# donydchen/matchnerf

Hardware: AMD Instinct MI355X
Metric: rendered rays/sec (3-view, 64 samples/ray) (higher is better)
Workload: dtype f32; 1 GPU

## Files before the change

matchnerf_amd/csrc/api.cpp:

```cpp
#include <string.h>
#include <stdarg.h>
#include <stdio.h>
#include <stdlib.h>

#include <mutex>

#include "common.hpp"
#include "launch_plan.hpp"

static thread_local char g_err[512] = "";

void mnerf_set_error(const char* fmt, ...) {
  va_list ap;
  va_start(ap, fmt);
  vsnprintf(g_err, sizeof(g_err), fmt, ap);
  va_end(ap);
}

extern "C" int mnerf_abi_version(void) { return MNERF_ABI_VERSION; }
extern "C" const char* mnerf_last_error(void) { return g_err; }

extern "C" int64_t mnerf_struct_size(int32_t which) {
  switch (which) {
    case 0: return (int64_t)sizeof(mnerf_view);
// ... 43 lines not shown
  c.height = c.tgt_height = rays->height, c.width = c.tgt_width = rays->width;
  c.near_ = rays->near_, c.far_ = rays->far_;
  c.strat_u = rays->strat_u;
  *out = c;
  return MNERF_OK;
}

static int env_int(const char* name, int dflt) {
  const char* e = getenv(name);
  return (e && *e) ? atoi(e) : dflt;
}

static mnerf_tuning read_tuning() {
  mnerf_tuning t;
  t.decoder_grid = env_int("MNERF_DECODER_GRID", 512);
  t.decoder_stagger = env_int("MNERF_DECODER_STAGGER", 16);
  t.decoder_stagger_mode = env_int("MNERF_DECODER_STAGGER_MODE", 0);
  t.cv_variant = env_int("MNERF_CV_VARIANT", 3);
  t.cv_mm = env_int("MNERF_CV_MM", 1);
  t.cv_mm_spw = env_int("MNERF_CV_MM_SPW", 4);
  t.cv_uvpair = env_int("MNERF_CV_UVPAIR", -1);
  t.cv_pair_block = env_int("MNERF_CV_PAIR_BLOCK", -1);
  t.cv_grid = env_int("MNERF_CV_GRID", 0);
  t.wa_min4 = env_int("MNERF_WA_MIN4", 200);
  t.wa_xcd = env_int("MNERF_WA_XCD", 1);
  t.render_fused = env_int("MNERF_RENDER_FUSED", 0);
  t.decoder_pp = env_int("MNERF_DECODER_PP", 1);
  t.decoder_pp_grid = env_int("MNERF_DECODER_PP_GRID", 256);
  t.decoder_pp_max_s = env_int("MNERF_DECODER_PP_MAX_S", 256);
  return t;
}

static mnerf_tuning g_tuning = read_tuning();
static std::mutex g_tuning_lock;
mnerf_tuning mnerf_tune() {
  std::lock_guard<std::mutex> hold(g_tuning_lock);
  return g_tuning;
}

extern "C" int mnerf_debug_set_knob(const char* name, int value, int* old_value) {
  std::lock_guard<std::mutex> hold(g_tuning_lock);
  struct Knob { const char* name; int* slot; };
  const Knob knobs[] = {{"decoder_pp", &g_tuning.decoder_pp}, {"decoder_pp_grid", &g_tuning.decoder_pp_grid},
                        {"decoder_pp_max_s", &g_tuning.decoder_pp_max_s}, {"decoder_grid", &g_tuning.decoder_grid},
                        {"cv_variant", &g_tuning.cv_variant}, {"cv_mm", &g_tuning.cv_mm}, {"cv_mm_spw", &g_tuning.cv_mm_spw}, {"cv_uvpair", &g_tuning.cv_uvpair}, {"cv_pair_block", &g_tuning.cv_pair_block}, {"cv_grid", &g_tuning.cv_grid},
                        {"render_fused", &g_tuning.render_fused}, {"wa_min4", &g_tuning.wa_min4}};
  for (const Knob& k : knobs)
    if (name && strcmp(name, k.name) == 0) {
      if (old_value) *old_value = *k.slot;
      *k.slot = value;
      return MNERF_OK;
    }
  mnerf_set_error("mnerf_debug_set_knob: unknown knob '%s'", name ? name : "(null)");
  return MNERF_E_RANGE;
}

extern "C" int mnerf_debug_launch_plan(const char* what, const int64_t* args, int32_t n_args, int32_t* plan, int32_t n_plan) {
  MNERF_REQUIRE(what && args && plan, MNERF_E_NULL, "mnerf_debug_launch_plan: NULL argument");
  struct Planner { const char* name; int (*fn)(const int64_t*, int32_t, int32_t*, int32_t); };
  const Planner planners[] = {{"conv2d", mnerf_plan_conv2d}, {"conv_gemm", mnerf_plan_conv_gemm}, {"conv_wgrad", mnerf_plan_conv_wgrad},
                              {"instance_norm", mnerf_plan_instance_norm}, {"instance_norm_backward", mnerf_plan_instance_norm},
                              {"window_attention", mnerf_plan_window_attention}};
  for (const Planner& p : planners)
    if (strcmp(what, p.name) == 0) return p.fn(args, n_args, plan, n_plan);
  mnerf_set_error("mnerf_debug_launch_plan: unknown dispatcher '%s'", what);
  return MNERF_E_RANGE;
}

bool mnerf_once_per_device(std::atomic<unsigned long long>& mask) {
  int dev = 0;
  (void)hipGetDevice(&dev);
  const unsigned long long bit = 1ull << (dev & 63);
  return (mask.fetch_or(bit, std::memory_order_relaxed) & bit) == 0;
}
```

matchnerf_amd/csrc/qkv.hip:

```cpp
#include "wa_common.hpp"

#define QKV_NW 2
#define QKV_SEG_FLOATS (32 * 256)
#define QKV_C 128

struct QkvParams {
  const float* xq;
  const float* xkv;
  float* out[3];
  const float* wstream;
  int n_tokens, seq_len, n_seq, kv_swap;
  int ew[3];
};

__device__ __forceinline__ int qkv_load_split(const float* __restrict__ row, PartsH (&xp)[8]) {
  float x[64];
  float amax = 0.0f;
#pragma unroll
  for (int t = 0; t < 8; ++t) {
    const float4 a = *reinterpret_cast<const float4*>(row + 16 * t), b = *reinterpret_cast<const float4*>(row + 16 * t + 4);
    x[8 * t + 0] = a.x; x[8 * t + 1] = a.y; x[8 * t + 2] = a.z; x[8 * t + 3] = a.w;
    x[8 * t + 4] = b.x; x[8 * t + 5] = b.y; x[8 * t + 6] = b.z; x[8 * t + 7] = b.w;
  }
#pragma unroll
// ... 76 lines not shown
  const float* xkv;
  float* q;
  u32x4* img;
  int* rec;
  const float* wstream;
  WinGeom G;
  int n_batch, n_tiles, total_tiles, kv_swap;
  int ew[3];
};

template <int NS>
__device__ __forceinline__ void ksteps_presplit_swapped(f32x16 (&acc)[4], unsigned base_lds, int lane, const PartsH* x) {
  lds_u32x4_cptr a = (lds_u32x4_cptr)(size_t)base_lds + lane;
  u32x4 ch = a[0], cl = a[64];
#pragma unroll
  for (int u = 0; u < NS; ++u) {
#pragma unroll
    for (int m = 0; m < 4; ++m) {
      const int i = u * 4 + m;
      const int nx = (i + 1 < NS * 4) ? (i + 1) * 128 : i * 128;
      const u32x4 nh = a[nx], nl = a[nx + 64];
      __builtin_amdgcn_sched_barrier(0);
      const f16x8 wh = __builtin_bit_cast(f16x8, ch), wl = __builtin_bit_cast(f16x8, cl);
      acc[m] = mfma16h(x[u].lo, wh, acc[m]);
      acc[m] = mfma16h(x[u].hi, wl, acc[m]);
      acc[m] = mfma16h(x[u].hi, wh, acc[m]);
      __builtin_amdgcn_sched_barrier(0);
      ch = nh;
      cl = nl;
    }
  }
}

__global__ __launch_bounds__(QKV_NW * 64, 2) void qkv_images_kernel(QkvImgParams P) {
  extern __shared__ __attribute__((aligned(16))) float qkv_smem[];
  const unsigned buf0 = (unsigned)(size_t)(__attribute__((address_space(3))) float*)qkv_smem;
  const int tid = threadIdx.x, lane = tid & 63;
  const int wave = __builtin_amdgcn_readfirstlane(tid >> 6);
  const int n = lane & 31, hl = lane >> 5;
  auto stage = [&](int seg) {
    const float* src = P.wstream + (size_t)seg * QKV_SEG_FLOATS + lane * 4;
    const unsigned dst = buf0 + (unsigned)(seg & 1) * (QKV_SEG_FLOATS * 4u);
    glds_segment(src, dst, QKV_SEG_FLOATS / 256, wave, QKV_NW);
  };
  stage(0);

  const WinGeom& G = P.G;
  const int t_raw = blockIdx.x * QKV_NW + wave;
  const bool tile_ok = t_raw < P.total_tiles;
  const int tile = tile_ok ? t_raw : P.total_tiles - 1;
  const int gwin = tile / P.n_tiles, kt = tile - gwin * P.n_tiles;
  const int n_win = G.splits * G.splits;
  const int b = gwin / n_win, win = gwin - b * n_win;
  const int wy = win / G.splits, wx = win - wy * G.splits;
  const int li = kt * WA_KT + n;
  const bool key_ok = li < G.Lw;
  int region_unused;
  const int tok = win_token(G, wy, wx, key_ok ? li : G.Lw - 1, region_unused);
  int b_kv = b;
  if (P.kv_swap) {
    b_kv = b + (P.n_batch >> 1);
    if (b_kv >= P.n_batch) b_kv -= P.n_batch;
  }
  const size_t hw = (size_t)G.h * G.w;
  const bool same_rows = !P.kv_swap && P.xkv == P.xq;

  PartsH xp[8];
  int eg = qkv_load_split(P.xq + ((size_t)b * hw + tok) * QKV_C + 8 * hl, xp);
  segment_wait();
  __syncthreads();

  u32x4* img = P.img + (size_t)tile * (WA_IMG_BYTES / 16) + lane;
  int ek = 0, ev = 0;
  int seg = 0;
#pragma unroll 1
  for (int proj = 0; proj < 3; ++proj) {
    if (proj == 1 && !same_rows) eg = qkv_load_split(P.xkv + ((size_t)b_kv * hw + tok) * QKV_C + 8 * hl, xp);
    f32x16 acc[4];
#pragma unroll
    for (int m = 0; m < 4; ++m) acc[m] = (f32x16)(0.0f);
#pragma unroll
    for (int half = 0; half < 2; ++half, ++seg) {
      if (seg + 1 < 6) stage(seg + 1);
      const unsigned cur = buf0 + (unsigned)(seg & 1) * (QKV_SEG_FLOATS * 4u);
      if (proj == 2) ksteps_presplit_swapped<4>(acc, cur, lane, xp + 4 * half);
      else ksteps_presplit<4, 4>(acc, cur, lane, xp + 4 * half);
      segment_wait();
      __syncthreads();
    }
    if (proj == 0) {
      if (tile_ok && key_ok) {
        const float cm = pow2i(-(P.ew[0] + eg));
        float* dst = P.q + ((size_t)b * hw + tok) * QKV_C + 4 * hl;
#pragma unroll
        for (int m = 0; m < 4; ++m)
#pragma unroll
          for (int g = 0; g < 4; ++g)
            *reinterpret_cast<float4*>(dst + 32 * m + 8 * g) =
                make_float4(acc[m][4 * g] * cm, acc[m][4 * g + 1] * cm, acc[m][4 * g + 2] * cm, acc[m][4 * g + 3] * cm);
      }
      continue;
    }
    if (proj == 1) {
      const float cm = pow2i(-(P.ew[1] + eg));
#pragma unroll
      for (int m = 0; m < 4; ++m)
#pragma unroll
        for (int r = 0; r < 16; ++r) acc[m][r] *= cm;
    } else {
#pragma unroll
      for (int r = 0; r < 16; ++r) {
        const int key = (r & 3) + 8 * (r >> 2) + 4 * hl;
        const int eg_key = __shfl(eg, key, 64);
        const float cm = pow2i(-(P.ew[2] + eg_key));
#pragma unroll
        for (int m = 0; m < 4; ++m) acc[m][r] *= cm;
      }
    }
    float tmax = 0.0f;
#pragma unroll
    for (int m = 0; m < 4; ++m)
#pragma unroll
      for (int r = 0; r < 16; ++r) tmax = fmaxf(tmax, fabsf(acc[m][r]));
#pragma unroll
    for (int off = 32; off > 0; off >>= 1) tmax = fmaxf(tmax, __shfl_xor(tmax, off, 64));
    const int et = gain_exp(tmax);
    const float mt = pow2i(et);
    if (proj == 1) {
      ek = et;
      if (tile_ok) {
#pragma unroll
        for (int t = 0; t < 8; ++t) {
          float v8[8];
#pragma unroll
          for (int j = 0; j < 8; ++j) v8[j] = acc[t >> 1][8 * (t & 1) + j];
          const PartsH kp = split8h(v8, mt);
          img[(2 * t) * 64] = __builtin_bit_cast(u32x4, kp.hi);
          img[(2 * t + 1) * 64] = __builtin_bit_cast(u32x4, kp.lo);
        }
      }
    } else {
      ev = et;
      if (tile_ok) {
#pragma unroll
        for (int t = 0; t < 2; ++t)
#pragma unroll
          for (int m = 0; m < 4; ++m) {
            float v8[8];
#pragma unroll
            for (int j = 0; j < 8; ++j) v8[j] = acc[m][8 * t + j];
            const PartsH vp = split8h(v8, mt);
            img[(WA_IMG_VOFF / 64 + 2 * (4 * t + m)) * 64] = __builtin_bit_cast(u32x4, vp.hi);
            img[(WA_IMG_VOFF / 64 + 2 * (4 * t + m) + 1) * 64] = __builtin_bit_cast(u32x4, vp.lo);
          }
      }
    }
  }
  if (tile_ok) {
    int* rec = P.rec + WA_REC_INTS * (size_t)tile;
    wa_store_regions(G, wy, wx, kt, lane, rec);
    if (lane == 0) {
      rec[0] = ek;
      rec[1] = ev;
    }
  }
}

extern "C" int mnerf_qkv_window_images(const float* wstream, const int32_t* ew, const float* x_q, const float* x_kv,
                                       int32_t kv_swap, float* q, void* workspace, size_t workspace_bytes, int32_t batch,
                                       int32_t h, int32_t w, int32_t num_splits, int32_t shifted, void* stream) {
  const char* who = "mnerf_qkv_window_images";
  WinGeom G;
  int do_shift;
  if (const int rc = wa_geometry(who, batch, h, w, num_splits, shifted, G, do_shift)) return rc;
  MNERF_REQUIRE(!kv_swap || batch % 2 == 0, MNERF_E_RANGE, "%s: kv_swap needs an even number of sequences, got %d", who, batch);
  if (batch == 0) return MNERF_OK;
  MNERF_REQUIRE(wstream && ew && x_q && x_kv && q, MNERF_E_NULL, "%s: NULL buffer", who);
  MNERF_REQUIRE(mnerf_aligned16(wstream) && mnerf_aligned16(x_q) && mnerf_aligned16(x_kv) && mnerf_aligned16(q), MNERF_E_ALIGN,
                "%s: buffers must be 16-byte aligned", who);
  const size_t need = wa_workspace_bytes(batch, h, w, num_splits);
  MNERF_REQUIRE(workspace && mnerf_aligned16(workspace), MNERF_E_ALIGN, "%s: workspace NULL or not 16-byte aligned", who);
  MNERF_REQUIRE(workspace_bytes >= need, MNERF_E_RANGE, "%s: workspace %zu bytes < %zu", who, workspace_bytes, need);
  QkvImgParams p;
  p.xq = x_q;
  p.xkv = x_kv;
  p.q = q;
  p.wstream = wstream;
  p.G = G;
  p.n_batch = batch;
  p.n_tiles = (G.Lw + WA_KT - 1) / WA_KT;
  p.total_tiles = batch * num_splits * num_splits * p.n_tiles;
  p.kv_swap = kv_swap ? 1 : 0;
  p.img = reinterpret_cast<u32x4*>(workspace);
  p.rec = reinterpret_cast<int*>(reinterpret_cast<char*>(workspace) + (size_t)p.total_tiles * WA_IMG_BYTES);
  for (int i = 0; i < 3; ++i) p.ew[i] = ew[i];
  const size_t lds = 2 * QKV_SEG_FLOATS * sizeof(float);
  static std::atomic<unsigned long long> attr{0};
  if (mnerf_once_per_device(attr))
    (void)hipFuncSetAttribute((const void*)qkv_images_kernel, hipFuncAttributeMaxDynamicSharedMemorySize, (int)lds);
  hipLaunchKernelGGL(qkv_images_kernel, dim3((p.total_tiles + QKV_NW - 1) / QKV_NW), dim3(QKV_NW * 64), lds, (hipStream_t)stream, p);
  return mnerf_check_launch(who);
}

extern "C" int64_t mnerf_qkv_wstream_floats(void) { return 6 * (int64_t)QKV_SEG_FLOATS; }

extern "C" int mnerf_qkv_projection(const float* wstream, const int32_t* ew, const float* x_q, const float* x_kv,
                                    int32_t kv_swap, float* q, float* k, float* v, int32_t n_seq, int32_t seq_len,
                                    void* stream) {
  const char* who = "mnerf_qkv_projection";
  MNERF_REQUIRE(n_seq >= 0 && seq_len >= 1 && (long long)n_seq * seq_len <= 0x7fffffffLL, MNERF_E_RANGE,
                "%s: n_seq=%d seq_len=%d", who, n_seq, seq_len);
  MNERF_REQUIRE(!kv_swap || n_seq % 2 == 0, MNERF_E_RANGE, "%s: kv_swap needs an even number of sequences, got %d", who, n_seq);
  if (n_seq == 0) return MNERF_OK;
  MNERF_REQUIRE(wstream && ew && x_q && x_kv && q && k && v, MNERF_E_NULL, "%s: NULL buffer", who);
  MNERF_REQUIRE(mnerf_aligned16(wstream) && mnerf_aligned16(x_q) && mnerf_aligned16(x_kv) && mnerf_aligned16(q) &&
                    mnerf_aligned16(k) && mnerf_aligned16(v),
                MNERF_E_ALIGN, "%s: buffers must be 16-byte aligned", who);
  QkvParams p;
  p.xq = x_q;
  p.xkv = x_kv;
  p.out[0] = q;
  p.out[1] = k;
  p.out[2] = v;
  p.wstream = wstream;
  p.n_tokens = n_seq * seq_len;
  p.seq_len = seq_len;
  p.n_seq = n_seq;
  p.kv_swap = kv_swap ? 1 : 0;
  for (int i = 0; i < 3; ++i) p.ew[i] = ew[i];
  const size_t lds = 2 * QKV_SEG_FLOATS * sizeof(float);
  static std::atomic<unsigned long long> attr{0};
  if (mnerf_once_per_device(attr))
    (void)hipFuncSetAttribute((const void*)qkv_kernel, hipFuncAttributeMaxDynamicSharedMemorySize, (int)lds);
// ... 5 lines not shown
```

matchnerf_amd/csrc/wa_common.hpp:

```cpp
#pragma once
#include "split_f16.hpp"

#define WA_C 128
#define WA_KT 32
#define WA_IMG_BYTES 32768
#define WA_IMG_VOFF 1024
#define WA_REC_INTS 8

struct WinGeom {
  int h, w, wh, ww, sh, sw, splits, Lw;
};

__device__ __forceinline__ int win_token(const WinGeom& G, int wy, int wx, int li, int& region) {
  const int ly = li / G.ww, lx = li - ly * G.ww;
  const int ry = wy * G.wh + ly, rx = wx * G.ww + lx;
  int oy = ry + G.sh, ox = rx + G.sw;
  if (oy >= G.h) oy -= G.h;
  if (ox >= G.w) ox -= G.w;
  const int regy = (ry >= G.h - G.wh) + (ry >= G.h - G.sh);
  const int regx = (rx >= G.w - G.ww) + (rx >= G.w - G.sw);
  region = regy * 3 + regx;
  return oy * G.w + ox;
}

__device__ __forceinline__ void wa_store_regions(const WinGeom& G, int wy, int wx, int kt, int lane, int* rec) {
  const int n = lane & 31;
  int li = kt * WA_KT + n, region;
  if (li >= G.Lw) li = G.Lw - 1;
  (void)win_token(G, wy, wx, li, region);
  unsigned nib = (unsigned)region << (4 * (n & 7));
  nib |= __shfl_xor(nib, 1, 64);
  nib |= __shfl_xor(nib, 2, 64);
  nib |= __shfl_xor(nib, 4, 64);
  if (lane < 32 && (lane & 7) == 0) rec[2 + (lane >> 3)] = (int)nib;
}

static inline int wa_geometry(const char* who, int32_t batch, int32_t h, int32_t w, int32_t num_splits, int32_t shifted,
                       WinGeom& G, int& do_shift) {
  MNERF_REQUIRE(batch >= 0 && h >= 1 && w >= 1 && num_splits >= 1, MNERF_E_RANGE, "%s: batch=%d h=%d w=%d splits=%d",
                who, batch, h, w, num_splits);
  MNERF_REQUIRE(h % num_splits == 0 && w % num_splits == 0, MNERF_E_RANGE, "%s: %dx%d not divisible into %d splits",
                who, h, w, num_splits);
  MNERF_REQUIRE(batch <= 65535 && num_splits * num_splits <= 65535, MNERF_E_RANGE, "%s: grid too large", who);
  G.h = h;
// ... 19 lines not shown
```

matchnerf_amd/csrc/window_attention.hip:

```cpp
#include <stdlib.h>

#include "wa_common.hpp"
#include "launch_plan.hpp"

__device__ __forceinline__ void wa_glds16(const float* gsrc, unsigned lds_byte_addr) {
  unsigned keep;
  asm volatile(
      "s_mov_b32 %0, m0\n\t"
      "s_mov_b32 m0, %2\n\t"
      "s_nop 0\n\t"
      "global_load_lds_dwordx4 %1, off\n\t"
      "s_mov_b32 m0, %0"
      : "=&s"(keep)
      : "v"(gsrc), "s"(lds_byte_addr)
      : "memory");
}

__device__ __forceinline__ void wa_glds16x4(const float* gsrc, unsigned lds_byte_addr) {
  unsigned keep;
  asm volatile(
      "s_mov_b32 %0, m0\n\t"
      "s_mov_b32 m0, %2\n\t"
      "s_nop 0\n\t"
      "global_load_lds_dwordx4 %1, off\n\t"
// ... 465 lines not shown
      for (int r = 0; r < 16; ++r) o[m][r] *= corr;
#pragma unroll
    for (int t = 0; t < 2; ++t) {
      float pv[8];
#pragma unroll
      for (int j = 0; j < 8; ++j) pv[j] = s[8 * t + j];
      const PartsH pp = split8h(pv, 16384.0f);
#pragma unroll
      for (int m = 0; m < 4; ++m) {
        const PartsH vp = split8h(vv[t][m], mv);
        o[m] = mfma16h(vp.hi, pp.lo, o[m]);
        o[m] = mfma16h(vp.lo, pp.hi, o[m]);
        o[m] = mfma16h(vp.hi, pp.hi, o[m]);
      }
    }
    asm volatile("s_waitcnt vmcnt(0)" ::: "memory");
    __syncthreads();
  }
  if (q_ok) {
    const float inv_l = pow2i(-(ev_run + 14)) / l_run;
    float* dst = out + seq_base + (size_t)q_tok * WA_C;
#pragma unroll
    for (int m = 0; m < 4; ++m)
#pragma unroll
      for (int g4 = 0; g4 < 4; ++g4) {
        const float4 t = make_float4(o[m][4 * g4] * inv_l, o[m][4 * g4 + 1] * inv_l,
                                     o[m][4 * g4 + 2] * inv_l, o[m][4 * g4 + 3] * inv_l);
        *reinterpret_cast<float4*>(dst + m * 32 + 8 * g4 + 4 * hl) = t;
      }
  }
}


__global__ __launch_bounds__(64) void wa_presplit_kernel(const float* __restrict__ k, const float* __restrict__ v,
                                                         u32x4* __restrict__ img, int* __restrict__ gains, WinGeom G) {
  const int lane = threadIdx.x, n = lane & 31, hl = lane >> 5;
  const int kt = blockIdx.x, win = blockIdx.y, b = blockIdx.z;
  const int wy = win / G.splits, wx = win - wy * G.splits;
  const size_t seq_base = (size_t)b * G.h * G.w * WA_C;
  const size_t tile = ((size_t)b * gridDim.y + win) * gridDim.x + kt;
  u32x4* dst = img + tile * (WA_IMG_BYTES / 16) + lane;
  int reg_unused;
  int ek, ev;
  {
    int li = kt * WA_KT + n;
    if (li >= G.Lw) li = G.Lw - 1;
    const int tok = win_token(G, wy, wx, li, reg_unused);
    const float4* src = reinterpret_cast<const float4*>(k + seq_base + (size_t)tok * WA_C + hl * 8);
    float kv[64];
    float kmax = 0.0f;
#pragma unroll
    for (int t = 0; t < 8; ++t) {
      const float4 a = src[4 * t], c = src[4 * t + 1];
      kv[8 * t + 0] = a.x; kv[8 * t + 1] = a.y; kv[8 * t + 2] = a.z; kv[8 * t + 3] = a.w;
      kv[8 * t + 4] = c.x; kv[8 * t + 5] = c.y; kv[8 * t + 6] = c.z; kv[8 * t + 7] = c.w;
    }
#pragma unroll
    for (int i = 0; i < 64; ++i) kmax = fmaxf(kmax, fabsf(kv[i]));
#pragma unroll
    for (int off = 32; off > 0; off >>= 1) kmax = fmaxf(kmax, __shfl_xor(kmax, off, 64));
    ek = gain_exp(kmax);
    const float mk = pow2i(ek);
#pragma unroll
    for (int t = 0; t < 8; ++t) {
      float v8[8];
#pragma unroll
      for (int j = 0; j < 8; ++j) v8[j] = kv[8 * t + j];
      const PartsH kp = split8h(v8, mk);
      dst[(2 * t) * 64] = __builtin_bit_cast(u32x4, kp.hi);
      dst[(2 * t + 1) * 64] = __builtin_bit_cast(u32x4, kp.lo);
    }
  }
  {
    float vv[2][4][8];
    float vmax = 0.0f;
#pragma unroll
    for (int t = 0; t < 2; ++t)
#pragma unroll
      for (int j = 0; j < 8; ++j) {
        const int r = 8 * t + j;
        int li = kt * WA_KT + (r & 3) + 8 * (r >> 2) + 4 * hl;
        if (li >= G.Lw) li = G.Lw - 1;
        const int tok = win_token(G, wy, wx, li, reg_unused);
        const float* row = v + seq_base + (size_t)tok * WA_C + n;
#pragma unroll
        for (int m = 0; m < 4; ++m) {
          const float x = row[32 * m];
          vv[t][m][j] = x;
          vmax = fmaxf(vmax, fabsf(x));
        }
      }
#pragma unroll
    for (int off = 32; off > 0; off >>= 1) vmax = fmaxf(vmax, __shfl_xor(vmax, off, 64));
    ev = gain_exp(vmax);
    const float mv = pow2i(ev);
#pragma unroll
    for (int t = 0; t < 2; ++t)
#pragma unroll
      for (int m = 0; m < 4; ++m) {
        const PartsH vp = split8h(vv[t][m], mv);
        dst[(WA_IMG_VOFF / 64 + 2 * (4 * t + m)) * 64] = __builtin_bit_cast(u32x4, vp.hi);
        dst[(WA_IMG_VOFF / 64 + 2 * (4 * t + m) + 1) * 64] = __builtin_bit_cast(u32x4, vp.lo);
      }
  }
  int* rec = gains + WA_REC_INTS * tile;
  wa_store_regions(G, wy, wx, kt, lane, rec);
  if (lane == 0) {
    rec[0] = ek;
    rec[1] = ev;
  }
}

__device__ __forceinline__ void wa_halves(float x, float& lo, float& hi) {
  unsigned a = __builtin_bit_cast(unsigned, x), b = a;
  asm("s_nop 1\n\tv_permlane32_swap_b32_e32 %0, %1" : "+v"(a), "+v"(b));
  lo = __builtin_bit_cast(float, a);
  hi = __builtin_bit_cast(float, b);
}

template <int NQW>
__device__ __forceinline__ void wa_stage_image(const u32x4* __restrict__ img_tile, unsigned lds_base, int wave, int lane) {
  for (int piece = wave; piece < WA_IMG_BYTES / 1024; piece += NQW)
    wa_glds16(reinterpret_cast<const float*>(img_tile + piece * 64 + lane),
              __builtin_amdgcn_readfirstlane(lds_base + (unsigned)piece * 1024u));
}

template <int NQW, bool STATS = false>
__global__ __launch_bounds__(NQW * 64, 2) void window_attention_pre_kernel(
    const float* __restrict__ q, const u32x4* __restrict__ img, const int* __restrict__ gains,
    float* __restrict__ out, WinGeom G, int shifted, float scale, int n_batch, int xcd_map, unsigned long long* tl) {
  extern __shared__ __attribute__((aligned(16))) float wa_smem[];
  const unsigned smem0 = (unsigned)(size_t)(__attribute__((address_space(3))) float*)wa_smem;
  const int tid = threadIdx.x, lane = tid & 63;
  const int wave = __builtin_amdgcn_readfirstlane(tid >> 6);
  const int n = lane & 31, hl = lane >> 5;
  const int n_win = G.splits * G.splits;
// ... 217 lines not shown
    WA_STAMP(5);
    ra = ra_next;
    rb = rb_next;
  }
#undef WA_SLOT
#ifdef MNERF_TIMELINE
  if (tl && lane == 0 && blockIdx.x < 64)
    for (int i = 0; i < 6; ++i) tl[(blockIdx.x * NQW + wave) * 6 + i] = tph[i];
#endif
  if (q_ok) {
    const float inv_l = pow2i(-(ev_run + 14)) / l_run;
    float* dst = out + seq_base + (size_t)q_tok * WA_C;
#pragma unroll
    for (int m = 0; m < 4; ++m)
#pragma unroll
      for (int g4 = 0; g4 < 4; ++g4) {
        const float4 t = make_float4(o[m][4 * g4] * inv_l, o[m][4 * g4 + 1] * inv_l,
                                     o[m][4 * g4 + 2] * inv_l, o[m][4 * g4 + 3] * inv_l);
        *reinterpret_cast<float4*>(dst + m * 32 + 8 * g4 + 4 * hl) = t;
      }
#ifndef MNERF_TIMELINE
    if constexpr (STATS) {
      if (hl == 0) {
        float* st = reinterpret_cast<float*>(tl);
        const size_t tok = (size_t)b * G.h * G.w + q_tok, n_tok = (size_t)n_batch * G.h * G.w;
        st[tok] = m_run;
        st[n_tok + tok] = l_run;
      }
    }
#endif
  }
}

extern "C" size_t mnerf_window_attention_workspace_bytes(int32_t batch, int32_t h, int32_t w, int32_t num_splits) {
  return wa_workspace_bytes(batch, h, w, num_splits);
}

static bool wa_take_four(int Lw, int n_win, int batch) {
  const long long wgs4 = (long long)((Lw + 127) / 128) * n_win * batch;
  return wgs4 >= mnerf_tune().wa_min4;
}

int mnerf_plan_window_attention(const int64_t* a, int32_t n_args, int32_t* plan, int32_t n_plan) {
  const char* who = "mnerf_debug_launch_plan(window_attention)";
  MNERF_REQUIRE(n_args == 4 && n_plan >= 1, MNERF_E_RANGE, "%s: takes 4 arguments and fills 1 value, got %d and %d", who, n_args, n_plan);
  MNERF_REQUIRE(a[0] >= 1 && a[0] <= 65535 && a[1] >= 1 && a[2] >= 1 && a[1] <= 0x7fff && a[2] <= 0x7fff && a[3] >= 1 && a[3] <= 255,
                MNERF_E_RANGE, "%s: batch=%lld h=%lld w=%lld splits=%lld", who, (long long)a[0], (long long)a[1], (long long)a[2], (long long)a[3]);
  MNERF_REQUIRE(a[1] % a[3] == 0 && a[2] % a[3] == 0, MNERF_E_RANGE, "%s: %lldx%lld not divisible into %lld splits", who, (long long)a[1],
                (long long)a[2], (long long)a[3]);
  plan[0] = wa_take_four((int)((a[1] / a[3]) * (a[2] / a[3])), (int)(a[3] * a[3]), (int)a[0]) ? 4 : 2;
  return MNERF_OK;
}

static int wa_launch_main(const char* who, const float* q, float* out, const WinGeom& G, int do_shift, int32_t batch,
                          int32_t num_splits, void* workspace, hipStream_t st, float* row_stats = nullptr) {
  const int n_tiles = (G.Lw + WA_KT - 1) / WA_KT;
  const int n_win = num_splits * num_splits;
  const u32x4* img = reinterpret_cast<const u32x4*>(workspace);
  const int* gains = reinterpret_cast<const int*>(reinterpret_cast<const char*>(workspace) + (size_t)batch * n_win * n_tiles * WA_IMG_BYTES);
  const float scale = 1.0f / sqrtf((float)WA_C);
  const size_t lds = 2 * WA_IMG_BYTES;
  static std::atomic<unsigned long long> attr{0};
  if (mnerf_once_per_device(attr)) {
    (void)hipFuncSetAttribute((const void*)window_attention_pre_kernel<4>, hipFuncAttributeMaxDynamicSharedMemorySize, (int)lds);
    (void)hipFuncSetAttribute((const void*)window_attention_pre_kernel<2>, hipFuncAttributeMaxDynamicSharedMemorySize, (int)lds);
    (void)hipFuncSetAttribute((const void*)window_attention_pre_kernel<4, true>, hipFuncAttributeMaxDynamicSharedMemorySize, (int)lds);
    (void)hipFuncSetAttribute((const void*)window_attention_pre_kernel<2, true>, hipFuncAttributeMaxDynamicSharedMemorySize, (int)lds);
  }
  unsigned long long* tl = nullptr;
#ifdef MNERF_TIMELINE
  if (const char* e = getenv("MNERF_WA_TIMELINE_PTR")) tl = (unsigned long long*)strtoull(e, nullptr, 0);
#endif
  const long long win_groups = ((long long)n_win * batch + 7) / 8;
  const int xcd = mnerf_tune().wa_xcd;
  const bool four = wa_take_four(G.Lw, n_win, batch);
  const int n_qb = four ? (G.Lw + 127) / 128 : (G.Lw + 63) / 64;
  const dim3 grid((unsigned)(8 * win_groups * n_qb));
#ifndef MNERF_TIMELINE
  if (row_stats) {
    unsigned long long* sp = reinterpret_cast<unsigned long long*>(row_stats);
    if (four)
      hipLaunchKernelGGL((window_attention_pre_kernel<4, true>), grid, dim3(256), lds, st, q, img, gains, out, G, do_shift, scale, batch, xcd, sp);
    else
      hipLaunchKernelGGL((window_attention_pre_kernel<2, true>), grid, dim3(128), lds, st, q, img, gains, out, G, do_shift, scale, batch, xcd, sp);
    return mnerf_check_launch(who);
  }
#else
  MNERF_REQUIRE(!row_stats, MNERF_E_UNSUPPORTED, "%s: no row statistics in the timeline build", who);
#endif
  if (four)
    hipLaunchKernelGGL(window_attention_pre_kernel<4>, grid, dim3(256), lds, st, q, img, gains, out, G, do_shift, scale, batch, xcd, tl);
  else
    hipLaunchKernelGGL(window_attention_pre_kernel<2>, grid, dim3(128), lds, st, q, img, gains, out, G, do_shift, scale, batch, xcd, tl);
  return mnerf_check_launch(who);
}

static int wa_check_workspace(const char* who, const void* workspace, size_t workspace_bytes, int32_t batch, int32_t h,
                              int32_t w, int32_t num_splits) {
  const size_t need = wa_workspace_bytes(batch, h, w, num_splits);
  MNERF_REQUIRE(workspace && mnerf_aligned16(workspace), MNERF_E_ALIGN, "%s: workspace NULL or not 16-byte aligned", who);
  MNERF_REQUIRE(workspace_bytes >= need, MNERF_E_RANGE, "%s: workspace %zu bytes < %zu", who, workspace_bytes, need);
  return MNERF_OK;
}

static int wa_presplit_impl(const char* who, const float* q, const float* k, const float* v, float* out, float* row_stats,
                            int32_t batch, int32_t h, int32_t w, int32_t num_splits, int32_t shifted, void* workspace,
                            size_t workspace_bytes, void* stream) {
  MNERF_REQUIRE(q && k && v && out, MNERF_E_NULL, "%s: NULL buffer", who);
  MNERF_REQUIRE(mnerf_aligned16(q) && mnerf_aligned16(k) && mnerf_aligned16(v) && mnerf_aligned16(out), MNERF_E_ALIGN,
                "%s: buffers must be 16-byte aligned", who);
  WinGeom G;
  int do_shift;
  if (const int rc = wa_geometry(who, batch, h, w, num_splits, shifted, G, do_shift)) return rc;
  if (batch == 0) return MNERF_OK;
  if (const int rc = wa_check_workspace(who, workspace, workspace_bytes, batch, h, w, num_splits)) return rc;
  const int n_tiles = (G.Lw + WA_KT - 1) / WA_KT;
  const int n_win = num_splits * num_splits;
  u32x4* img = reinterpret_cast<u32x4*>(workspace);
  int* gains = reinterpret_cast<int*>(reinterpret_cast<char*>(workspace) + (size_t)batch * n_win * n_tiles * WA_IMG_BYTES);
  hipStream_t st = (hipStream_t)stream;
  hipLaunchKernelGGL(wa_presplit_kernel, dim3(n_tiles, n_win, batch), dim3(64), 0, st, k, v, img, gains, G);
  return wa_launch_main(who, q, out, G, do_shift, batch, num_splits, workspace, st, row_stats);
}

extern "C" int mnerf_window_attention_presplit(const float* q, const float* k, const float* v, float* out,
                                               int32_t batch, int32_t h, int32_t w, int32_t num_splits, int32_t shifted,
                                               void* workspace, size_t workspace_bytes, void* stream) {
  return wa_presplit_impl("mnerf_window_attention_presplit", q, k, v, out, nullptr, batch, h, w, num_splits, shifted, workspace,
                          workspace_bytes, stream);
}

extern "C" int mnerf_window_attention_presplit_stats(const float* q, const float* k, const float* v, float* out, float* row_stats,
                                                     int32_t batch, int32_t h, int32_t w, int32_t num_splits, int32_t shifted,
                                                     void* workspace, size_t workspace_bytes, void* stream) {
  const char* who = "mnerf_window_attention_presplit_stats";
  MNERF_REQUIRE(row_stats, MNERF_E_NULL, "%s: row_stats is NULL", who);
  return wa_presplit_impl(who, q, k, v, out, row_stats, batch, h, w, num_splits, shifted, workspace, workspace_bytes, stream);
}

extern "C" int mnerf_window_attention_images(const float* q, float* out, int32_t batch, int32_t h, int32_t w,
                                             int32_t num_splits, int32_t shifted, const void* workspace,
                                             size_t workspace_bytes, void* stream) {
  const char* who = "mnerf_window_attention_images";
  MNERF_REQUIRE(q && out, MNERF_E_NULL, "%s: NULL buffer", who);
  MNERF_REQUIRE(mnerf_aligned16(q) && mnerf_aligned16(out), MNERF_E_ALIGN, "%s: buffers must be 16-byte aligned", who);
  WinGeom G;
  int do_shift;
  if (const int rc = wa_geometry(who, batch, h, w, num_splits, shifted, G, do_shift)) return rc;
  if (batch == 0) return MNERF_OK;
  if (const int rc = wa_check_workspace(who, workspace, workspace_bytes, batch, h, w, num_splits)) return rc;
  return wa_launch_main(who, q, out, G, do_shift, batch, num_splits, const_cast<void*>(workspace), (hipStream_t)stream);
}

extern "C" int mnerf_window_attention(const float* q, const float* k, const float* v, float* out,
                                      int32_t batch, int32_t h, int32_t w, int32_t num_splits,
                                      int32_t shifted, int32_t math, void* stream) {
  MNERF_REQUIRE(q && k && v && out, MNERF_E_NULL, "mnerf_window_attention: NULL buffer");
  MNERF_REQUIRE(mnerf_aligned16(q) && mnerf_aligned16(k) && mnerf_aligned16(v) && mnerf_aligned16(out),
                MNERF_E_ALIGN, "mnerf_window_attention: buffers must be 16-byte aligned");
  MNERF_REQUIRE(batch >= 0 && h >= 1 && w >= 1 && num_splits >= 1, MNERF_E_RANGE,
                "mnerf_window_attention: batch=%d h=%d w=%d splits=%d", batch, h, w, num_splits);
  MNERF_REQUIRE(h % num_splits == 0 && w % num_splits == 0, MNERF_E_RANGE,
                "mnerf_window_attention: %dx%d not divisible into %d splits", h, w, num_splits);
  MNERF_REQUIRE(batch <= 65535 && num_splits * num_splits <= 65535, MNERF_E_RANGE,
                "mnerf_window_attention: grid too large");
  MNERF_REQUIRE(math == MNERF_WA_SPLIT_BF16 || math == MNERF_WA_EXACT_F32 || math == MNERF_WA_SPLIT_F16, MNERF_E_UNSUPPORTED,
                "mnerf_window_attention: math=%d", math);
  if (batch == 0) return MNERF_OK;
  WinGeom G;
  G.h = h;
  G.w = w;
  G.splits = num_splits;
  G.wh = h / num_splits;
  G.ww = w / num_splits;
  const int do_shift = (shifted && num_splits > 1) ? 1 : 0;
  G.sh = do_shift ? G.wh / 2 : 0;
  G.sw = do_shift ? G.ww / 2 : 0;
  G.Lw = G.wh * G.ww;
  const float scale = 1.0f / sqrtf((float)WA_C);
  hipStream_t st = (hipStream_t)stream;
  const size_t lds = 4 * WA_KT * WA_C * sizeof(float);
  const bool split = math == MNERF_WA_SPLIT_BF16;
  const bool split_h = math == MNERF_WA_SPLIT_F16;
  static std::atomic<unsigned long long> attr_f32{0}, attr_split{0}, attr_split_h{0};
// ... 32 lines not shown
```

Before: 13.21 million rays/s.

## Add 16-row MFMA window-attention kernel with matching K/V image layout

Adds a window-attention kernel that uses 16x16x32 f16 MFMA with 16-row query fragments instead of the prior 32-row form. The K/V image written by the presplit and QKV projection kernels gets a matching 16-row layout. The path is on by default (MNERF_WA_ROWS=16) whenever the 128-query workgroup path is chosen. The aim is better MFMA shape efficiency and finer-grained softmax reductions, at the cost of new layout code that every producer must keep consistent.

```diff
diff --git a/matchnerf_amd/csrc/api.cpp b/matchnerf_amd/csrc/api.cpp
--- a/matchnerf_amd/csrc/api.cpp
+++ b/matchnerf_amd/csrc/api.cpp
@@ -99,7 +99,12 @@
 }
 
 static mnerf_tuning g_tuning = read_tuning();
+static int g_wa_rows = env_int("MNERF_WA_ROWS", 16);
 static std::mutex g_tuning_lock;
+int mnerf_wa_rows() {
+  std::lock_guard<std::mutex> hold(g_tuning_lock);
+  return g_wa_rows;
+}
 mnerf_tuning mnerf_tune() {
   std::lock_guard<std::mutex> hold(g_tuning_lock);
   return g_tuning;
@@ -111,7 +116,7 @@
   const Knob knobs[] = {{"decoder_pp", &g_tuning.decoder_pp}, {"decoder_pp_grid", &g_tuning.decoder_pp_grid},
                         {"decoder_pp_max_s", &g_tuning.decoder_pp_max_s}, {"decoder_grid", &g_tuning.decoder_grid},
                         {"cv_variant", &g_tuning.cv_variant}, {"cv_mm", &g_tuning.cv_mm}, {"cv_mm_spw", &g_tuning.cv_mm_spw}, {"cv_uvpair", &g_tuning.cv_uvpair}, {"cv_pair_block", &g_tuning.cv_pair_block}, {"cv_grid", &g_tuning.cv_grid},
-                        {"render_fused", &g_tuning.render_fused}, {"wa_min4", &g_tuning.wa_min4}};
+                        {"render_fused", &g_tuning.render_fused}, {"wa_min4", &g_tuning.wa_min4}, {"wa_rows", &g_wa_rows}};
   for (const Knob& k : knobs)
     if (name && strcmp(name, k.name) == 0) {
       if (old_value) *old_value = *k.slot;
diff --git a/matchnerf_amd/csrc/qkv.hip b/matchnerf_amd/csrc/qkv.hip
--- a/matchnerf_amd/csrc/qkv.hip
+++ b/matchnerf_amd/csrc/qkv.hip
@@ -132,6 +132,7 @@
   }
 }
 
+template <int LAYOUT>
 __global__ __launch_bounds__(QKV_NW * 64, 2) void qkv_images_kernel(QkvImgParams P) {
   extern __shared__ __attribute__((aligned(16))) float qkv_smem[];
   const unsigned buf0 = (unsigned)(size_t)(__attribute__((address_space(3))) float*)qkv_smem;
@@ -170,7 +171,8 @@
   segment_wait();
   __syncthreads();
 
-  u32x4* img = P.img + (size_t)tile * (WA_IMG_BYTES / 16) + lane;
+  u32x4* img_tile = P.img + (size_t)tile * (WA_IMG_BYTES / 16);
+  u32x4* img = img_tile + lane;
   int ek = 0, ev = 0;
   int seg = 0;
 #pragma unroll 1
@@ -235,8 +237,14 @@
 #pragma unroll
           for (int j = 0; j < 8; ++j) v8[j] = acc[t >> 1][8 * (t & 1) + j];
           const PartsH kp = split8h(v8, mt);
-          img[(2 * t) * 64] = __builtin_bit_cast(u32x4, kp.hi);
-          img[(2 * t + 1) * 64] = __builtin_bit_cast(u32x4, kp.lo);
+          if constexpr (LAYOUT == WA_IMG_ROWS16) {
+            u32x4* dst = img_tile + (2 * (4 * (n >> 4) + (t >> 1))) * 64 + (n & 15) + 16 * (2 * (t & 1) + hl);
+            dst[0] = __builtin_bit_cast(u32x4, kp.hi);
+            dst[64] = __builtin_bit_cast(u32x4, kp.lo);
+          } else {
+            img[(2 * t) * 64] = __builtin_bit_cast(u32x4, kp.hi);
+            img[(2 * t + 1) * 64] = __builtin_bit_cast(u32x4, kp.lo);
+          }
         }
       }
     } else {
@@ -247,11 +255,20 @@
 #pragma unroll
           for (int m = 0; m < 4; ++m) {
             float v8[8];
-#pragma unroll
-            for (int j = 0; j < 8; ++j) v8[j] = acc[m][8 * t + j];
-            const PartsH vp = split8h(v8, mt);
-            img[(WA_IMG_VOFF / 64 + 2 * (4 * t + m)) * 64] = __builtin_bit_cast(u32x4, vp.hi);
-            img[(WA_IMG_VOFF / 64 + 2 * (4 * t + m) + 1) * 64] = __builtin_bit_cast(u32x4, vp.lo);
+            if constexpr (LAYOUT == WA_IMG_ROWS16) {
+#pragma unroll
+              for (int j = 0; j < 8; ++j) v8[j] = acc[m][8 * (j >> 2) + 4 * t + (j & 3)];
+              const PartsH vp = split8h(v8, mt);
+              u32x4* dst = img_tile + (WA_IMG_VOFF / 64 + 2 * (2 * m + (n >> 4))) * 64 + (n & 15) + 16 * (2 * t + hl);
+              dst[0] = __builtin_bit_cast(u32x4, vp.hi);
+              dst[64] = __builtin_bit_cast(u32x4, vp.lo);
+            } else {
+#pragma unroll
+              for (int j = 0; j < 8; ++j) v8[j] = acc[m][8 * t + j];
+              const PartsH vp = split8h(v8, mt);
+              img[(WA_IMG_VOFF / 64 + 2 * (4 * t + m)) * 64] = __builtin_bit_cast(u32x4, vp.hi);
+              img[(WA_IMG_VOFF / 64 + 2 * (4 * t + m) + 1) * 64] = __builtin_bit_cast(u32x4, vp.lo);
+            }
           }
       }
     }
@@ -296,9 +313,15 @@
   for (int i = 0; i < 3; ++i) p.ew[i] = ew[i];
   const size_t lds = 2 * QKV_SEG_FLOATS * sizeof(float);
   static std::atomic<unsigned long long> attr{0};
-  if (mnerf_once_per_device(attr))
-    (void)hipFuncSetAttribute((const void*)qkv_images_kernel, hipFuncAttributeMaxDynamicSharedMemorySize, (int)lds);
-  hipLaunchKernelGGL(qkv_images_kernel, dim3((p.total_tiles + QKV_NW - 1) / QKV_NW), dim3(QKV_NW * 64), lds, (hipStream_t)stream, p);
+  if (mnerf_once_per_device(attr)) {
+    (void)hipFuncSetAttribute((const void*)qkv_images_kernel<WA_IMG_ROWS32>, hipFuncAttributeMaxDynamicSharedMemorySize, (int)lds);
+    (void)hipFuncSetAttribute((const void*)qkv_images_kernel<WA_IMG_ROWS16>, hipFuncAttributeMaxDynamicSharedMemorySize, (int)lds);
+  }
+  const dim3 grid((p.total_tiles + QKV_NW - 1) / QKV_NW);
+  if (wa_rows16(G.Lw, num_splits * num_splits, batch))
+    hipLaunchKernelGGL(qkv_images_kernel<WA_IMG_ROWS16>, grid, dim3(QKV_NW * 64), lds, (hipStream_t)stream, p);
+  else
+    hipLaunchKernelGGL(qkv_images_kernel<WA_IMG_ROWS32>, grid, dim3(QKV_NW * 64), lds, (hipStream_t)stream, p);
   return mnerf_check_launch(who);
 }
 
diff --git a/matchnerf_amd/csrc/wa_common.hpp b/matchnerf_amd/csrc/wa_common.hpp
--- a/matchnerf_amd/csrc/wa_common.hpp
+++ b/matchnerf_amd/csrc/wa_common.hpp
@@ -7,9 +7,19 @@
 #define WA_IMG_VOFF 1024
 #define WA_REC_INTS 8
 
+enum { WA_IMG_ROWS32 = 0, WA_IMG_ROWS16 = 1 };
+
 struct WinGeom {
   int h, w, wh, ww, sh, sw, splits, Lw;
 };
+
+static inline bool wa_take_four(int Lw, int n_win, int batch) {
+  const long long wgs4 = (long long)((Lw + 127) / 128) * n_win * batch;
+  return wgs4 >= mnerf_tune().wa_min4;
+}
+
+int mnerf_wa_rows();
+static inline bool wa_rows16(int Lw, int n_win, int batch) { return mnerf_wa_rows() != 32 && wa_take_four(Lw, n_win, batch); }
 
 __device__ __forceinline__ int win_token(const WinGeom& G, int wy, int wx, int li, int& region) {
   const int ly = li / G.ww, lx = li - ly * G.ww;
diff --git a/matchnerf_amd/csrc/window_attention.hip b/matchnerf_amd/csrc/window_attention.hip
--- a/matchnerf_amd/csrc/window_attention.hip
+++ b/matchnerf_amd/csrc/window_attention.hip
@@ -521,9 +521,11 @@
 }
 
 
+template <int LAYOUT>
 __global__ __launch_bounds__(64) void wa_presplit_kernel(const float* __restrict__ k, const float* __restrict__ v,
                                                          u32x4* __restrict__ img, int* __restrict__ gains, WinGeom G) {
   const int lane = threadIdx.x, n = lane & 31, hl = lane >> 5;
+  const int c16 = lane & 15, g16 = lane >> 4;
   const int kt = blockIdx.x, win = blockIdx.y, b = blockIdx.z;
   const int wy = win / G.splits, wx = win - wy * G.splits;
   const size_t seq_base = (size_t)b * G.h * G.w * WA_C;
@@ -532,17 +534,34 @@
   int reg_unused;
   int ek, ev;
   {
-    int li = kt * WA_KT + n;
-    if (li >= G.Lw) li = G.Lw - 1;
-    const int tok = win_token(G, wy, wx, li, reg_unused);
-    const float4* src = reinterpret_cast<const float4*>(k + seq_base + (size_t)tok * WA_C + hl * 8);
     float kv[64];
     float kmax = 0.0f;
-#pragma unroll
-    for (int t = 0; t < 8; ++t) {
-      const float4 a = src[4 * t], c = src[4 * t + 1];
-      kv[8 * t + 0] = a.x; kv[8 * t + 1] = a.y; kv[8 * t + 2] = a.z; kv[8 * t + 3] = a.w;
-      kv[8 * t + 4] = c.x; kv[8 * t + 5] = c.y; kv[8 * t + 6] = c.z; kv[8 * t + 7] = c.w;
+    if constexpr (LAYOUT == WA_IMG_ROWS16) {
+#pragma unroll
+      for (int kb = 0; kb < 2; ++kb) {
+        int li = kt * WA_KT + 16 * kb + c16;
+        if (li >= G.Lw) li = G.Lw - 1;
+        const int tok = win_token(G, wy, wx, li, reg_unused);
+        const float4* src = reinterpret_cast<const float4*>(k + seq_base + (size_t)tok * WA_C + g16 * 8);
+#pragma unroll
+        for (int T = 0; T < 4; ++T) {
+          const float4 a = src[8 * T], c = src[8 * T + 1];
+          const int f = 4 * kb + T;
+          kv[8 * f + 0] = a.x; kv[8 * f + 1] = a.y; kv[8 * f + 2] = a.z; kv[8 * f + 3] = a.w;
+          kv[8 * f + 4] = c.x; kv[8 * f + 5] = c.y; kv[8 * f + 6] = c.z; kv[8 * f + 7] = c.w;
+        }
+      }
+    } else {
+      int li = kt * WA_KT + n;
+      if (li >= G.Lw) li = G.Lw - 1;
+      const int tok = win_token(G, wy, wx, li, reg_unused);
+      const float4* src = reinterpret_cast<const float4*>(k + seq_base + (size_t)tok * WA_C + hl * 8);
+#pragma unroll
+      for (int t = 0; t < 8; ++t) {
+        const float4 a = src[4 * t], c = src[4 * t + 1];
+        kv[8 * t + 0] = a.x; kv[8 * t + 1] = a.y; kv[8 * t + 2] = a.z; kv[8 * t + 3] = a.w;
+        kv[8 * t + 4] = c.x; kv[8 * t + 5] = c.y; kv[8 * t + 6] = c.z; kv[8 * t + 7] = c.w;
+      }
     }
 #pragma unroll
     for (int i = 0; i < 64; ++i) kmax = fmaxf(kmax, fabsf(kv[i]));
@@ -561,21 +580,25 @@
     }
   }
   {
-    float vv[2][4][8];
+    float vv[8][8];
     float vmax = 0.0f;
 #pragma unroll
     for (int t = 0; t < 2; ++t)
 #pragma unroll
       for (int j = 0; j < 8; ++j) {
         const int r = 8 * t + j;
-        int li = kt * WA_KT + (r & 3) + 8 * (r >> 2) + 4 * hl;
+        int li;
+        if constexpr (LAYOUT == WA_IMG_ROWS16)
+          li = kt * WA_KT + 16 * (j >> 2) + 4 * g16 + (j & 3);
+        else
+          li = kt * WA_KT + (r & 3) + 8 * (r >> 2) + 4 * hl;
         if (li >= G.Lw) li = G.Lw - 1;
         const int tok = win_token(G, wy, wx, li, reg_unused);
-        const float* row = v + seq_base + (size_t)tok * WA_C + n;
+        const float* row = v + seq_base + (size_t)tok * WA_C + (LAYOUT == WA_IMG_ROWS16 ? 64 * t + c16 : n);
 #pragma unroll
         for (int m = 0; m < 4; ++m) {
-          const float x = row[32 * m];
-          vv[t][m][j] = x;
+          const float x = row[LAYOUT == WA_IMG_ROWS16 ? 16 * m : 32 * m];
+          vv[4 * t + m][j] = x;
           vmax = fmaxf(vmax, fabsf(x));
         }
       }
@@ -584,13 +607,11 @@
     ev = gain_exp(vmax);
     const float mv = pow2i(ev);
 #pragma unroll
-    for (int t = 0; t < 2; ++t)
-#pragma unroll
-      for (int m = 0; m < 4; ++m) {
-        const PartsH vp = split8h(vv[t][m], mv);
-        dst[(WA_IMG_VOFF / 64 + 2 * (4 * t + m)) * 64] = __builtin_bit_cast(u32x4, vp.hi);
-        dst[(WA_IMG_VOFF / 64 + 2 * (4 * t + m) + 1) * 64] = __builtin_bit_cast(u32x4, vp.lo);
-      }
+    for (int f = 0; f < 8; ++f) {
+      const PartsH vp = split8h(vv[f], mv);
+      dst[(WA_IMG_VOFF / 64 + 2 * f) * 64] = __builtin_bit_cast(u32x4, vp.hi);
+      dst[(WA_IMG_VOFF / 64 + 2 * f + 1) * 64] = __builtin_bit_cast(u32x4, vp.lo);
+    }
   }
   int* rec = gains + WA_REC_INTS * tile;
   wa_store_regions(G, wy, wx, kt, lane, rec);
@@ -874,14 +895,232 @@
   }
 }
 
+typedef v4f32 f32x4;
+
+__device__ __forceinline__ f32x4 mfma32h(f16x8 a, f16x8 b, f32x4 c) { return __builtin_amdgcn_mfma_f32_16x16x32_f16(a, b, c, 0, 0, 0); }
+
+__device__ __forceinline__ void wa_row_pair(float x, float& even, float& odd) {
+  unsigned a = __builtin_bit_cast(unsigned, x), b = a;
+  asm("s_nop 1\n\tv_permlane16_swap_b32_e32 %0, %1" : "+v"(a), "+v"(b));
+  even = __builtin_bit_cast(float, a);
+  odd = __builtin_bit_cast(float, b);
+}
+__device__ __forceinline__ float wa_quad_max(float x) {
+  float a, b;
+  wa_row_pair(x, a, b);
+  x = fmaxf(a, b);
+  wa_halves(x, a, b);
+  return fmaxf(a, b);
+}
+__device__ __forceinline__ float wa_quad_sum(float x) {
+  float a, b;
+  wa_row_pair(x, a, b);
+  x = a + b;
+  wa_halves(x, a, b);
+  return a + b;
+}
+
+#define WA16_NW 8
+template <bool STATS = false>
+__global__ __launch_bounds__(WA16_NW * 64, 2) void window_attention_pre16_kernel(
+    const float* __restrict__ q, const u32x4* __restrict__ img, const int* __restrict__ gains,
+    float* __restrict__ out, WinGeom G, int shifted, float scale, int n_batch, int xcd_map, float* __restrict__ row_stats) {
+  extern __shared__ __attribute__((aligned(16))) float wa_smem[];
+  const unsigned smem0 = (unsigned)(size_t)(__attribute__((address_space(3))) float*)wa_smem;
+  const int tid = threadIdx.x, lane = tid & 63;
+  const int wave = __builtin_amdgcn_readfirstlane(tid >> 6);
+  const int n = lane & 15, g = lane >> 4;
+  const int n_win = G.splits * G.splits;
+  const int n_qb = (G.Lw + WA16_NW * 16 - 1) / (WA16_NW * 16);
+  const int slot = xcd_map ? blockIdx.x >> 3 : blockIdx.x, wl = slot / n_qb;
+  const int qblock = slot - wl * n_qb, gwin = xcd_map ? wl * 8 + (blockIdx.x & 7) : wl;
+  if (gwin >= n_win * n_batch) return;
+  const int b = gwin / n_win, win = gwin - b * n_win;
+  const int wy = win / G.splits, wx = win - wy * G.splits;
+  const size_t seq_base = (size_t)b * G.h * G.w * WA_C;
+
+  const int n_tiles = (G.Lw + WA_KT - 1) / WA_KT;
+  const size_t tile0 = (size_t)gwin * n_tiles;
+  const u32x4* img_win = img + tile0 * (WA_IMG_BYTES / 16);
+  const int4* rec_win = reinterpret_cast<const int4*>(gains + WA_REC_INTS * tile0);
+  wa_stage_image<WA16_NW>(img_win, smem0, wave, lane);
+  int4 ra = rec_win[0], rb = rec_win[1];
+
+  const int qi_raw = (qblock * WA16_NW + wave) * 16 + n;
+  const bool q_ok = qi_raw < G.Lw;
+  int q_region;
+  const int q_tok = win_token(G, wy, wx, q_ok ? qi_raw : (G.Lw - 1), q_region);
+  PartsH qp[4];
+  int eq;
+  {
+    const float4* src = reinterpret_cast<const float4*>(q + seq_base + (size_t)q_tok * WA_C + g * 8);
+    float qv[32];
+    float qmax = 0.0f;
+#pragma unroll
+    for (int T = 0; T < 4; ++T) {
+      const float4 a = src[8 * T], c = src[8 * T + 1];
+      qv[8 * T + 0] = a.x; qv[8 * T + 1] = a.y; qv[8 * T + 2] = a.z; qv[8 * T + 3] = a.w;
+      qv[8 * T + 4] = c.x; qv[8 * T + 5] = c.y; qv[8 * T + 6] = c.z; qv[8 * T + 7] = c.w;
+    }
+#pragma unroll
+    for (int i = 0; i < 32; ++i) qmax = fmaxf(qmax, fabsf(qv[i]));
+    qmax = wa_quad_max(qmax);
+    eq = gain_exp(qmax);
+    const float mq = pow2i(eq);
+#pragma unroll
+    for (int T = 0; T < 4; ++T) {
+      float v8[8];
+#pragma unroll
+      for (int j = 0; j < 8; ++j) v8[j] = qv[8 * T + j];
+      qp[T] = split8h(v8, mq);
+    }
+  }
+  f32x4 o[8];
+#pragma unroll
+  for (int m = 0; m < 8; ++m) o[m] = (f32x4)(0.0f);
+  float m_run = -3.0e38f, l_run = 0.0f;
+  int ev_run = 0;
+
+  asm volatile("s_waitcnt vmcnt(0)" ::: "memory");
+  __syncthreads();
+
+  const float l2e = 1.44269504088896f;
+  const float mask_l2 = -100.0f * l2e;
+  const bool ragged = (G.Lw & (WA_KT - 1)) != 0;
+  const unsigned q_rep = (unsigned)q_region * 0x11111111u;
+  for (int kt = 0; kt < n_tiles; ++kt) {
+    const int cur = kt & 1;
+    const int ktn = kt + 1 < n_tiles ? kt + 1 : kt;
+    const int ek = ra.x, ev = ra.y;
+    lds_u32x4_cptr frag = (lds_u32x4_cptr)(size_t)(smem0 + (unsigned)cur * WA_IMG_BYTES) + lane;
+    f32x4 sa[2][2];
+#pragma unroll
+    for (int kb = 0; kb < 2; ++kb)
+#pragma unroll
+      for (int a = 0; a < 2; ++a) sa[kb][a] = (f32x4)(0.0f);
+    f16x8 khi[2][2][2], klo[2][2][2];
+#pragma unroll
+    for (int tp = 0; tp < 2; ++tp)
+#pragma unroll
+      for (int kb = 0; kb < 2; ++kb)
+#pragma unroll
+        for (int a = 0; a < 2; ++a) {
+          const int f = 4 * kb + 2 * tp + a;
+          klo[tp][kb][a] = __builtin_bit_cast(f16x8, frag[(2 * f + 1) * 64]);
+          khi[tp][kb][a] = __builtin_bit_cast(f16x8, frag[(2 * f) * 64]);
+        }
+#define WA16_DMA()                                                                                                          \
+  do {                                                         \
+    const int piece = wave * 4;                                                                                             \
+    wa_glds16x4(reinterpret_cast<const float*>(img_win + (size_t)ktn * (WA_IMG_BYTES / 16) + lane + piece * 64),            \
+                __builtin_amdgcn_readfirstlane(smem0 + (unsigned)(cur ^ 1) * WA_IMG_BYTES + (unsigned)piece * 1024u));      \
+  } while (0)
+    WA16_DMA();
+    __builtin_amdgcn_sched_barrier(0);
+#pragma unroll
+    for (int tp = 0; tp < 2; ++tp) {
+#pragma unroll
+      for (int kb = 0; kb < 2; ++kb)
+#pragma unroll
+        for (int a = 0; a < 2; ++a) sa[kb][a] = mfma32h(klo[tp][kb][a], qp[2 * tp + a].hi, sa[kb][a]);
+#pragma unroll
+      for (int kb = 0; kb < 2; ++kb)
+#pragma unroll
+        for (int a = 0; a < 2; ++a) sa[kb][a] = mfma32h(khi[tp][kb][a], qp[2 * tp + a].lo, sa[kb][a]);
+#pragma unroll
+      for (int kb = 0; kb < 2; ++kb)
+#pragma unroll
+        for (int a = 0; a < 2; ++a) sa[kb][a] = mfma32h(khi[tp][kb][a], qp[2 * tp + a].hi, sa[kb][a]);
+    }
+    f16x8 vhi[8], vlo[8];
+#pragma unroll
+    for (int m = 0; m < 8; ++m) {
+      vlo[m] = __builtin_bit_cast(f16x8, frag[(WA_IMG_VOFF / 64 + 2 * m + 1) * 64]);
+      vhi[m] = __builtin_bit_cast(f16x8, frag[(WA_IMG_VOFF / 64 + 2 * m) * 64]);
+    }
+    const int4 ra_next = rec_win[2 * ktn], rb_next = rec_win[2 * ktn + 1];
+    __builtin_amdgcn_sched_barrier(0);
+    const float sscale = scale * l2e * pow2i(-(ek + eq));
+    float s[8];
+#pragma unroll
+    for (int kb = 0; kb < 2; ++kb) {
+      const f32x4 sum = sa[kb][0] + sa[kb][1];
+#pragma unroll
+      for (int r = 0; r < 4; ++r) s[4 * kb + r] = sum[r] * sscale;
+    }
+    if (shifted) {
+      const unsigned w0 = (g & 2) ? (unsigned)ra.w : (unsigned)ra.z, w1 = (g & 2) ? (unsigned)rb.y : (unsigned)rb.x;
+      const unsigned sh = 16u * (unsigned)(g & 1);
+      const unsigned x = (((w0 >> sh) & 0xffffu) | ((w1 >> sh) << 16)) ^ q_rep;
+#pragma unroll
+      for (int j = 0; j < 8; ++j)
+        if ((x >> (4 * j)) & 15u) s[j] += mask_l2;
+    }
+    if (ragged && kt == n_tiles - 1) {
+#pragma unroll
+      for (int j = 0; j < 8; ++j)
+        if (kt * WA_KT + 16 * (j >> 2) + 4 * g + (j & 3) >= G.Lw) s[j] = -3.0e38f;
+    }
+    float tmax = s[0];
+#pragma unroll
+    for (int j = 1; j < 8; ++j) tmax = fmaxf(tmax, s[j]);
+    tmax = wa_quad_max(tmax);
+    const float m_new = fmaxf(m_run, tmax);
+    const float alpha = __builtin_amdgcn_exp2f(m_run - m_new);
+    float psum = 0.0f;
+#pragma unroll
+    for (int j = 0; j < 8; ++j) {
+      const float p = __builtin_amdgcn_exp2f(s[j] - m_new);
+      s[j] = p;
+      psum += p;
+    }
+    psum = wa_quad_sum(psum);
+    l_run = l_run * alpha + psum;
+    m_run = m_new;
+    const float corr = alpha * pow2i(ev - ev_run);
+    ev_run = ev;
+    if (__builtin_amdgcn_ballot_w64(corr != 1.0f) != 0) {
+#pragma unroll
+      for (int m = 0; m < 8; ++m)
+#pragma unroll
+        for (int r = 0; r < 4; ++r) o[m][r] *= corr;
+    }
+    const PartsH pp = split8h(s, 16384.0f);
+#pragma unroll
+    for (int mh = 0; mh < 2; ++mh) {
+#pragma unroll
+      for (int m = 0; m < 4; ++m) o[4 * mh + m] = mfma32h(vlo[4 * mh + m], pp.hi, o[4 * mh + m]);
+#pragma unroll
+      for (int m = 0; m < 4; ++m) o[4 * mh + m] = mfma32h(vhi[4 * mh + m], pp.lo, o[4 * mh + m]);
+#pragma unroll
+      for (int m = 0; m < 4; ++m) o[4 * mh + m] = mfma32h(vhi[4 * mh + m], pp.hi, o[4 * mh + m]);
+    }
+    asm volatile("s_waitcnt vmcnt(0)" ::: "memory");
+    __syncthreads();
+    ra = ra_next;
+    rb = rb_next;
+  }
+#undef WA16_DMA
+  if (q_ok) {
+    const float inv_l = pow2i(-(ev_run + 14)) / l_run;
+    float* dst = out + seq_base + (size_t)q_tok * WA_C + 4 * g;
+#pragma unroll
+    for (int m = 0; m < 8; ++m)
+      *reinterpret_cast<float4*>(dst + 16 * m) = make_float4(o[m][0] * inv_l, o[m][1] * inv_l, o[m][2] * inv_l, o[m][3] * inv_l);
+    if constexpr (STATS) {
+      if (g == 0) {
+        const size_t tok = (size_t)b * G.h * G.w + q_tok, n_tok = (size_t)n_batch * G.h * G.w;
+        row_stats[tok] = m_run;
+        row_stats[n_tok + tok] = l_run;
+      }
+    }
+  }
+}
+
 extern "C" size_t mnerf_window_attention_workspace_bytes(int32_t batch, int32_t h, int32_t w, int32_t num_splits) {
   return wa_workspace_bytes(batch, h, w, num_splits);
 }
 
-static bool wa_take_four(int Lw, int n_win, int batch) {
-  const long long wgs4 = (long long)((Lw + 127) / 128) * n_win * batch;
-  return wgs4 >= mnerf_tune().wa_min4;
-}
 
 int mnerf_plan_window_attention(const int64_t* a, int32_t n_args, int32_t* plan, int32_t n_plan) {
   const char* who = "mnerf_debug_launch_plan(window_attention)";
@@ -890,12 +1129,14 @@
                 MNERF_E_RANGE, "%s: batch=%lld h=%lld w=%lld splits=%lld", who, (long long)a[0], (long long)a[1], (long long)a[2], (long long)a[3]);
   MNERF_REQUIRE(a[1] % a[3] == 0 && a[2] % a[3] == 0, MNERF_E_RANGE, "%s: %lldx%lld not divisible into %lld splits", who, (long long)a[1],
                 (long long)a[2], (long long)a[3]);
-  plan[0] = wa_take_four((int)((a[1] / a[3]) * (a[2] / a[3])), (int)(a[3] * a[3]), (int)a[0]) ? 4 : 2;
+  const int lw = (int)((a[1] / a[3]) * (a[2] / a[3])), n_win = (int)(a[3] * a[3]);
+  plan[0] = wa_take_four(lw, n_win, (int)a[0]) ? 4 : 2;
+  if (n_plan >= 2) plan[1] = wa_rows16(lw, n_win, (int)a[0]) ? 16 : 32;
   return MNERF_OK;
 }
 
 static int wa_launch_main(const char* who, const float* q, float* out, const WinGeom& G, int do_shift, int32_t batch,
-                          int32_t num_splits, void* workspace, hipStream_t st, float* row_stats = nullptr) {
+                          int32_t num_splits, void* workspace, hipStream_t st, bool rows16, float* row_stats = nullptr) {
   const int n_tiles = (G.Lw + WA_KT - 1) / WA_KT;
   const int n_win = num_splits * num_splits;
   const u32x4* img = reinterpret_cast<const u32x4*>(workspace);
@@ -908,6 +1149,8 @@
     (void)hipFuncSetAttribute((const void*)window_attention_pre_kernel<2>, hipFuncAttributeMaxDynamicSharedMemorySize, (int)lds);
     (void)hipFuncSetAttribute((const void*)window_attention_pre_kernel<4, true>, hipFuncAttributeMaxDynamicSharedMemorySize, (int)lds);
     (void)hipFuncSetAttribute((const void*)window_attention_pre_kernel<2, true>, hipFuncAttributeMaxDynamicSharedMemorySize, (int)lds);
+    (void)hipFuncSetAttribute((const void*)window_attention_pre16_kernel<false>, hipFuncAttributeMaxDynamicSharedMemorySize, (int)lds);
+    (void)hipFuncSetAttribute((const void*)window_attention_pre16_kernel<true>, hipFuncAttributeMaxDynamicSharedMemorySize, (int)lds);
   }
   unsigned long long* tl = nullptr;
 #ifdef MNERF_TIMELINE
@@ -918,6 +1161,14 @@
   const bool four = wa_take_four(G.Lw, n_win, batch);
   const int n_qb = four ? (G.Lw + 127) / 128 : (G.Lw + 63) / 64;
   const dim3 grid((unsigned)(8 * win_groups * n_qb));
+  if (rows16) {
+    MNERF_REQUIRE(four, MNERF_E_UNSUPPORTED, "%s: the 16-row instance is a form of the 128-query workgroups", who);
+    if (row_stats)
+      hipLaunchKernelGGL(window_attention_pre16_kernel<true>, grid, dim3(WA16_NW * 64), lds, st, q, img, gains, out, G, do_shift, scale, batch, xcd, row_stats);
+    else
+      hipLaunchKernelGGL(window_attention_pre16_kernel<false>, grid, dim3(WA16_NW * 64), lds, st, q, img, gains, out, G, do_shift, scale, batch, xcd, row_stats);
+    return mnerf_check_launch(who);
+  }
 #ifndef MNERF_TIMELINE
   if (row_stats) {
     unsigned long long* sp = reinterpret_cast<unsigned long long*>(row_stats);
@@ -961,8 +1212,12 @@
   u32x4* img = reinterpret_cast<u32x4*>(workspace);
   int* gains = reinterpret_cast<int*>(reinterpret_cast<char*>(workspace) + (size_t)batch * n_win * n_tiles * WA_IMG_BYTES);
   hipStream_t st = (hipStream_t)stream;
-  hipLaunchKernelGGL(wa_presplit_kernel, dim3(n_tiles, n_win, batch), dim3(64), 0, st, k, v, img, gains, G);
-  return wa_launch_main(who, q, out, G, do_shift, batch, num_splits, workspace, st, row_stats);
+  const bool rows16 = wa_rows16(G.Lw, n_win, batch);
+  if (rows16)
+    hipLaunchKernelGGL(wa_presplit_kernel<WA_IMG_ROWS16>, dim3(n_tiles, n_win, batch), dim3(64), 0, st, k, v, img, gains, G);
+  else
+    hipLaunchKernelGGL(wa_presplit_kernel<WA_IMG_ROWS32>, dim3(n_tiles, n_win, batch), dim3(64), 0, st, k, v, img, gains, G);
+  return wa_launch_main(who, q, out, G, do_shift, batch, num_splits, workspace, st, rows16, row_stats);
 }
 
 extern "C" int mnerf_window_attention_presplit(const float* q, const float* k, const float* v, float* out,
@@ -991,7 +1246,8 @@
   if (const int rc = wa_geometry(who, batch, h, w, num_splits, shifted, G, do_shift)) return rc;
   if (batch == 0) return MNERF_OK;
   if (const int rc = wa_check_workspace(who, workspace, workspace_bytes, batch, h, w, num_splits)) return rc;
-  return wa_launch_main(who, q, out, G, do_shift, batch, num_splits, const_cast<void*>(workspace), (hipStream_t)stream);
+  return wa_launch_main(who, q, out, G, do_shift, batch, num_splits, const_cast<void*>(workspace), (hipStream_t)stream,
+                        wa_rows16(G.Lw, num_splits * num_splits, batch));
 }
 
 extern "C" int mnerf_window_attention(const float* q, const float* k, const float* v, float* out,
```

Result: no change. 13.30 million rays/s, median of 6 (+0.7%).
